# facebookresearch/mbrl-lib

Hardware: AMD Instinct MI355X
Metric: candidate-steps/sec (pop×particles×horizon / plan) per CEM iter; plans/sec (higher is better)
Workload: dtype f32

## Files before the change

### __graft_entry__.py

```python
import os
import subprocess
import sys

ROOT = os.path.dirname(os.path.abspath(__file__))
PKG = os.path.join(ROOT, "mbrl-lib_amd")
CSRC = os.path.join(PKG, "csrc")
LIB = os.path.join(PKG, "hipets", "libhipets.so")
BUILDINFO = os.path.join(PKG, "hipets", "libhipets.buildinfo.json")
OBJDIR = os.path.join(PKG, "build")
HIPCC = os.environ.get("HIPCC", "/opt/rocm/bin/hipcc")
HOST_UNITS = ["train.hip", "plan.hip", "rollout.hip", "model.hip", "policy.hip", "sac.hip", "value.hip", "ensemble.hip", "policy_rollout.hip", "replay.hip", "comm.hip", "engine.hip"]
UNITS = ["rollout_r3.hip", "rollout_r4_gen.hip", "rollout_r4_gens.hip", "rollout_r3_gen.hip", "rollout_r3_gens.hip", "rollout_r2.hip", "rollout_r2_gen.hip",
         "rollout_r2_gens.hip", "rollout_r1_gen.hip", "rollout_r1_gens.hip", "rollout_r1.hip", "rollout_r4.hip", "rollout_r2_fast.hip", "rollout_r3_fast.hip",
         "rollout_r1_fast.hip", "planet.hip"] + HOST_UNITS + ["rollout_r4_fast.hip"]
FLAGS = ["--offload-arch=gfx950", "-O3", "-std=c++17", "-ffp-contract=off", "-fPIC", "-Wno-pass-failed"]


def _sources():
    return sorted(os.path.join(CSRC, f) for f in os.listdir(CSRC)) + [os.path.join(ROOT, "include", "hipets.h")]


def source_digest(extra_flags=()):
    import hashlib

# ... 108 lines not shown
            if asm and op.split("_")[0] in ("global", "buffer", "flat", "scratch") and re.search(r"_store_dwordx[34]", op):
                store_data = regs(ops[1]) if op.startswith(("global", "flat", "scratch")) else regs(ops[0])
            recent.append((nop, regs(ops[0]) if (op.startswith("v_") and ops) else set(), line, store_data))
        if len(recent) > 8:
            del recent[0]
        return inflight

    def undrained(inflight, recent):
        ws = 0
        for nop, written, _, store in reversed(recent[-3:]):
            if ws >= 2:
                break
            if nop is not None:
                ws += nop
                continue
            if written or store:
                return True
            ws += 1
        return bool(inflight)

    edges = []
    kernel, inflight, recent = "?", [], []
    for kind, text, asm in prog:
        if kind == "kernel":
            kernel, inflight, recent = text, [], []
        elif kind == "ins":
            inflight = step(kernel, text, asm, inflight, recent, True, "")
            op = text.split()[0]
            if op.startswith("s_cbranch") or op == "s_branch":
                target = text.split()[-1]
                if target in labels and undrained(inflight, recent):
                    edges.append((kernel, target, list(inflight), list(recent)))
            if op in ("s_branch", "s_endpgm", "s_setpc_b64"):
                inflight, recent = [], []
    done = set()
    for kernel, target, inflight, recent in edges:
        key = (target, tuple(sorted((tuple(sorted(r)), c) for r, c in inflight)), tuple(t[2] for t in recent[-3:]))
        if key in done:
            continue
        done.add(key)
        walked = 0
        for kind, text, asm in prog[labels[target]:]:
            if kind == "kernel" or walked >= 16:
                break
            if kind != "ins":
                continue
            inflight = step(kernel, text, asm, inflight, recent, False, f" (reached by a branch to {target})")
            walked += 1
            if text.split()[0] in ("s_branch", "s_endpgm", "s_setpc_b64"):
                break
    unique, base_seen = [], set()
    for f in findings:
        base = f.split(" (reached by a branch")[0]
        if base not in base_seen:
            base_seen.add(base)
            unique.append(f)
    return seen, unique


def parse_kernel_resources(asm_path):
    import re

    out, cur, meta = {}, None, None
    keys = {"NumVgprs": "VGPRs", "NumAgprs": "AGPRs", "ScratchSize": "ScratchSize [bytes/lane]", "Occupancy": "Occupancy [waves/SIMD]"}
    for line in open(asm_path, errors="replace"):
        m = re.match(r"^(\S+):\s+; @", line)
        if m:
            cur = m.group(1)
            continue
        m = re.match(r"^; (NumVgprs|NumAgprs|ScratchSize|Occupancy): (\d+)", line)
        if m and cur:
            out.setdefault(cur, {})[keys[m.group(1)]] = int(m.group(2))
            continue
        m = re.match(r"^\s+\.name:\s+(\S+)", line)
        if m:
            meta = m.group(1)
            continue
        m = re.match(r"^\s+\.(sgpr|vgpr)_spill_count:\s+(\d+)", line)
        if m and meta:
            out.setdefault(meta, {})["SGPRs Spill" if m.group(1) == "sgpr" else "VGPRs Spill"] = int(m.group(2))
    return {k: v for k, v in out.items() if "VGPRs" in v and "SGPRs Spill" in v}


def build_library(out=LIB, extra_flags=(), objdir=OBJDIR, force=False):
    import json
    from concurrent.futures import ThreadPoolExecutor

    digest = source_digest(extra_flags)
    if not force and built_digest(out) == digest:
        return digest
    os.makedirs(objdir, exist_ok=True)
    objs = [os.path.join(objdir, u.replace(".hip", ".o")) for u in UNITS]

    resources = {}
    isa = {"asm_mfmas": 0, "hazards": [], "units_scanned": []}

    def compile_unit(u, o):
        cmd = [HIPCC] + FLAGS + list(extra_flags) + ["-save-temps=obj", "-c", os.path.join(CSRC, u), "-o", o]
        print("[build]", " ".join(cmd), flush=True)
        proc = subprocess.run(cmd, stderr=subprocess.PIPE, text=True)
        for line in proc.stderr.splitlines():
            if "argument unused during compilation" not in line:
                print(line, file=sys.stderr)
        if proc.returncode != 0:
            raise subprocess.CalledProcessError(proc.returncode, cmd)
        stem = os.path.basename(o)[:-2]
        for f in os.listdir(objdir):
            if (f.startswith(stem + "-") or f.startswith(stem + ".")) and f != stem + ".o":
                path = os.path.join(objdir, f)
                if f.endswith("gfx950.s"):
                    resources.update(parse_kernel_resources(path))
                    n, found = scan_isa_hazards(path)
                    isa["asm_mfmas"] += n
                    isa["hazards"] += found
                    isa["units_scanned"].append(u)
                os.remove(path)

    with ThreadPoolExecutor(max_workers=min(len(UNITS), os.cpu_count() or 1)) as ex:
        list(ex.map(lambda uo: compile_unit(*uo), zip(UNITS, objs)))
    link_extra = [f for f in extra_flags if f.startswith("-fsanitize") or f in ("-fno-gpu-sanitize", "-shared-libsan")]
    cmd = [HIPCC, "--offload-arch=gfx950", "-shared", "-fPIC"] + link_extra + objs + ["-o", out]
    print("[build]", " ".join(cmd), flush=True)
    subprocess.run(cmd, check=True)
    with open(os.path.splitext(out)[0] + ".buildinfo.json", "w") as f:
        json.dump({"source_digest": digest, "flags": FLAGS + list(extra_flags), "units": UNITS, "kernels": resources, "isa": isa}, f)
    for h in isa["hazards"][:20]:
        print("[build] ISA HAZARD:", h, file=sys.stderr)
    if isa["hazards"] and not os.environ.get("HIPETS_ALLOW_ISA_HAZARDS") and "-O1" not in extra_flags:
        raise RuntimeError(f"{len(isa['hazards'])} ISA hazard finding(s) in {out}: see {os.path.splitext(out)[0]}.buildinfo.json")
    return digest


DEBUG_LIB = os.path.join(PKG, "hipets", "libhipets_debug.so")
ASAN_LIB = os.path.join(PKG, "hipets", "libhipets_asan.so")
DEBUG_OBJDIR = os.path.join(PKG, "build_debug")
DEBUG_FLAGS = ["-O1", "-gline-tables-only", "-DHIPETS_DEBUG_BOUNDS=1"]
ASAN_FLAGS = ["-fsanitize=address", "-fno-gpu-sanitize", "-shared-libsan", "-Wno-option-ignored"]


def asan_runtime() -> str:
    out = subprocess.run([HIPCC, "--print-file-name=libclang_rt.asan-x86_64.so"], capture_output=True, text=True).stdout.strip()
    if not os.path.isabs(out) or not os.path.exists(out):
        import glob

        found = sorted(glob.glob("/opt/rocm/lib/llvm/lib/clang/*/lib/linux/libclang_rt.asan-x86_64.so"))
        out = found[-1] if found else out
    return out


def build_debug(force: bool = False) -> str:
    import json

    digest = source_digest(DEBUG_FLAGS)
    rebuilt = built_digest(DEBUG_LIB) != digest or force
    build_library(out=DEBUG_LIB, extra_flags=DEBUG_FLAGS, objdir=DEBUG_OBJDIR, force=force)
    asan_digest = source_digest(DEBUG_FLAGS + ASAN_FLAGS)
    if rebuilt or built_digest(ASAN_LIB) != asan_digest:
        from concurrent.futures import ThreadPoolExecutor

        def compile_asan(u):
            obj = os.path.join(DEBUG_OBJDIR, u.replace(".hip", "_asan.o"))
            cmd = [HIPCC] + FLAGS + DEBUG_FLAGS + ASAN_FLAGS + ["-c", os.path.join(CSRC, u), "-o", obj]
            print("[build]", " ".join(cmd), flush=True)
            subprocess.run(cmd, check=True)
            return obj

        with ThreadPoolExecutor(max_workers=min(len(HOST_UNITS), os.cpu_count() or 1)) as ex:
            objs = list(ex.map(compile_asan, HOST_UNITS))
        others = [os.path.join(DEBUG_OBJDIR, u.replace(".hip", ".o")) for u in UNITS if u not in HOST_UNITS]
        cmd = [HIPCC, "--offload-arch=gfx950", "-shared", "-fPIC", "-fsanitize=address", "-fno-gpu-sanitize", "-shared-libsan"] + objs + others + ["-o", ASAN_LIB]
        print("[build]", " ".join(cmd), flush=True)
        subprocess.run(cmd, check=True)
        with open(os.path.splitext(ASAN_LIB)[0] + ".buildinfo.json", "w") as f:
            json.dump({"source_digest": asan_digest, "flags": FLAGS + DEBUG_FLAGS + ASAN_FLAGS, "units": UNITS}, f)
    return DEBUG_LIB


def build(force: bool = False, debug: bool = True) -> None:
    build_library(force=force)
    if debug and os.environ.get("HIPETS_BUILD_DEBUG", "1") != "0":
        build_debug(force)
    build_c_client(force)
    build_fake_rccl(force)
    build_residency_harness(force)
    build_resident_heads_harness(force)
    for p in (PKG, ROOT):
        if p not in sys.path:
            sys.path.insert(0, p)
    import hipets
    from hipets import _lib

    _lib.load()
    from oracle import pets_oracle

# ... 103 lines not shown
```

### mbrl-lib_amd/csrc/gemm_f32.hpp

```cpp
#pragma once
#include <type_traits>

#include "common.hpp"
#include "rollout_types.hpp"

namespace hipets {

__device__ __forceinline__ void mfma16x16x4(const float a, const float b, f32x4& c) {
    asm volatile("v_mfma_f32_16x16x4_f32 %0, %1, %2, %0" : "+v"(c) : "v"(a), "v"(b));
}
__device__ __forceinline__ void mfma16x16x4_ra(const float a, const float b, f32x4& c) {
    asm volatile("v_mfma_f32_16x16x4_f32 %0, %1, %2, %0" : "+v"(c) : "a"(a), "v"(b));
}
__device__ __forceinline__ void mfma_drain() { asm volatile("s_nop 15" ::: "memory"); }

__device__ __forceinline__ int lds_col(int c) { return (c & ~15) | ((c & 3) << 2) | ((c >> 2) & 3); }

constexpr int kProfCountShift = 44;
struct Prof {
    long long* slot;
    long long t;
    bool on;
    __device__ __forceinline__ void mark(int phase) {
        if (on) {
            const long long now = clock64();
            slot[phase] += (now - t) + (1ll << kProfCountShift);
            t = now;
        }
    }
};

#ifndef HIPETS_LEAN_PROF
#define HIPETS_LEAN_PROF 0
#endif

template <int R, int CT, int EX>
struct GemmFrags {
    f32x4 b[CT > 0 ? CT : 1];
    f32x4 bx[EX > 0 ? EX : 1];
    f32x4 a[R];
    f32x4 ax[EX > 0 ? EX : 1];
};

using u32x4g = __attribute__((ext_vector_type(4))) unsigned;

template <int R> struct MinWavesOf { static constexpr int value = R <= 2 ? 2 : 1; };

#ifndef HIPETS_DEBUG_BOUNDS
#define HIPETS_DEBUG_BOUNDS 0
#endif
#if HIPETS_DEBUG_BOUNDS
__host__ __device__ inline void hipets_bound_fail(const int line) {
#if defined(__HIP_DEVICE_COMPILE__)
    printf("hipets: bound violated at gemm_f32.hpp / rollout.hpp line %d (workgroup %d, thread %d)\n", line, (int)blockIdx.x, (int)threadIdx.x);
    __builtin_trap();
#else
    (void)line;
#endif
}
#define HIPETS_BOUND(cond) do { if (!(cond)) hipets_bound_fail(__LINE__); } while (0)
#else
#define HIPETS_BOUND(cond) ((void)0)
#endif

struct ResHead {
    f32x4 b[3], bx[3], bv[3], bvx[3];
};
__device__ __forceinline__ void res_load(f32x4& dst, const float* const p) { asm volatile("global_load_dwordx4 %0, %1, off" : "=a"(dst) : "v"(p) : "memory"); }
__device__ __forceinline__ void res_pin(f32x4& v) { asm volatile("" : "+a"(v)); }

struct NoTail {};
struct FusedSlot {
    float mxA, mxB, mnA, mnB, pA, pB;
    double nmA, nmB, nsA, nsB;
    int rid, ndA, ndB;
    float n0, n1;
};
template <class P, class D, class F, class G>
struct TailStages {
    P prep;
    D draw;
    F unit;
    G finish;
};
template <class P, class D, class F, class G>
__device__ __forceinline__ TailStages<P, D, F, G> make_tail(P p, D d, F f, G g) { return TailStages<P, D, F, G>{p, d, f, g}; }

__device__ __forceinline__ f32x4 silu4(const f32x4 a) {
    using f32x2 = __attribute__((ext_vector_type(2))) float;
    const f32x2 k = {-1.44269504088896340736f, -1.44269504088896340736f}, one = {1.0f, 1.0f};
    const f32x2 lo = {a[0], a[1]}, hi = {a[2], a[3]};
    f32x2 tl = lo * k, th = hi * k;
    tl[0] = __builtin_amdgcn_exp2f(tl[0]); tl[1] = __builtin_amdgcn_exp2f(tl[1]);
    th[0] = __builtin_amdgcn_exp2f(th[0]); th[1] = __builtin_amdgcn_exp2f(th[1]);
    tl = tl + one; th = th + one;
    tl[0] = __builtin_amdgcn_rcpf(tl[0]); tl[1] = __builtin_amdgcn_rcpf(tl[1]);
    th[0] = __builtin_amdgcn_rcpf(th[0]); th[1] = __builtin_amdgcn_rcpf(th[1]);
    const f32x2 yl = lo * tl, yh = hi * th;
    return f32x4{yl[0], yl[1], yh[0], yh[1]};
}

constexpr int kKsSlots = 4;
struct KsArgs {
    const float* part_in;
    float* part_out;
    int tile;
    int k0, n;
    int wave;
};

template <int R, int CT, int EX, int ACT, class TL = NoTail, int LD = -1, bool SPL = false, int KCS = -1, int KS = 0, int RES = 0>
__device__ __forceinline__ void wave_gemm(const float* __restrict__ in, float* __restrict__ out, const int ld_rt,
                                          const float* __restrict__ W, const float* __restrict__ bias, const int KC_rt,
                                          const int tail_steps, const int c_first, const Extras ex,
                                          const bool apply_act, const int act, const float slope, const int lane,
                                          Prof& prof, const TL* tl = nullptr, const int ldi_rt = 0, const KsArgs* ks = nullptr,
                                          const ResHead* rh = nullptr, const int rsel = 0) {
    static_assert(!RES || (LD > 0 && KS == 0 && R >= 3 && CT <= 3 && EX <= 3), "resident heads: shape-specialised one-wave-per-SIMD instances");
    constexpr int CTn = CT > 0 ? CT : 1;
    constexpr int EXn = EX > 0 ? EX : 1;
    constexpr bool KSI = (KS & 1) != 0, KSO = (KS & 2) != 0;
    static_assert(!KS || (R == 1 && LD > 0), "k-split: one-tile shape-specialised instances, rolled k loop");
    static_assert(!KSO || (std::is_same<TL, NoTail>::value && EX == 0 && !SPL), "k-split producer: a hidden op");
    f32x4 acc[CTn][R];
    f32x4 accx[EXn];
    const int ld = LD > 0 ? LD : ld_rt;
    const int ldi = ldi_rt > 0 ? ldi_rt : ld;
    const int KC = KCS > 0 ? KCS : KC_rt;

    const int exc[kMaxExtras] = {ex.c0, ex.c1, ex.c2, ex.c3};
    const int exr[kMaxExtras] = {ex.r0, ex.r1, ex.r2, ex.r3};
    unsigned woff[CTn], wxoff[EXn];
    int axoff[EXn];
#pragma unroll
    for (int ct = 0; ct < CT; ++ct) woff[ct] = (unsigned)(((c_first + kWaves * ct) * KC * 64 + lane) * 16);
#pragma unroll
    for (int e = 0; e < EX; ++e) {
        wxoff[e] = (unsigned)((exc[e] * KC * 64 + lane) * 16);
        axoff[e] = exr[e] * 16 * ldi;
    }
    const float* ap = in + (lane & 15) * ldi + 4 * (lane >> 4);
    f32x4 bv[CTn], bvx[EXn];
    if constexpr (!RES) {
#pragma unroll
    for (int ct = 0; ct < CT; ++ct) bv[ct] = *reinterpret_cast<const f32x4*>(bias + (c_first + kWaves * ct) * 16 + 4 * (lane >> 4));
#pragma unroll
    for (int e = 0; e < EX; ++e) bvx[e] = *reinterpret_cast<const f32x4*>(bias + exc[e] * 16 + 4 * (lane >> 4));
    }
    const unsigned long long wbits = reinterpret_cast<unsigned long long>(W);
    const unsigned long long wuni = ((unsigned long long)(unsigned)__builtin_amdgcn_readfirstlane((int)(wbits >> 32)) << 32) |
                                    (unsigned long long)(unsigned)__builtin_amdgcn_readfirstlane((int)(unsigned)wbits);
    const __amdgpu_buffer_rsrc_t wrsrc = __builtin_amdgcn_make_buffer_rsrc(reinterpret_cast<float*>(wuni), 0, 0x7FFFFFFF, 0x00020000);
    auto wload = [&](const unsigned voff, const int kk) __attribute__((always_inline)) {
        const u32x4g v = __builtin_amdgcn_raw_buffer_load_b128(wrsrc, (int)voff, kk * 1024, 0);
        f32x4 r;
        __builtin_memcpy(&r, &v, 16);
        return r;
    };
    auto load = [&](GemmFrags<R, CT, EX>& f, const int kk) __attribute__((always_inline)) {
#pragma unroll
        for (int ct = 0; ct < CT; ++ct) f.b[ct] = wload(woff[ct], kk);
#pragma unroll
        for (int e = 0; e < EX; ++e) f.bx[e] = wload(wxoff[e], kk);
#pragma unroll
        for (int r = 0; r < R; ++r) f.a[r] = *reinterpret_cast<const f32x4*>(ap + r * 16 * ldi + kk * 16);
#pragma unroll
        for (int e = 0; e < EX; ++e) f.ax[e] = *reinterpret_cast<const f32x4*>(ap + axoff[e] + kk * 16);
    };
    constexpr bool kSplit = (CT * R + EX) == 1;
    constexpr bool kSplitAll = SPL && !kSplit;
    f32x4 acc_odd = f32x4{0.f, 0.f, 0.f, 0.f};
    f32x4 acco[CTn][R], accxo[EXn];
#pragma unroll
    for (int ct = 0; ct < CTn; ++ct)
#pragma unroll
        for (int r = 0; r < R; ++r) acco[ct][r] = f32x4{0.f, 0.f, 0.f, 0.f};
#pragma unroll
    for (int e = 0; e < EXn; ++e) accxo[e] = f32x4{0.f, 0.f, 0.f, 0.f};
    auto kstep = [&](const GemmFrags<R, CT, EX>& f, const int s) __attribute__((always_inline)) {
        asm volatile("s_nop 1");
        if constexpr (kSplit) {
            f32x4& dst = (s & 1) ? acc_odd : (CT ? acc[0][0] : accx[0]);
            if constexpr (CT) mfma16x16x4(f.b[0][s], f.a[0][s], dst);
            else mfma16x16x4(f.bx[0][s], f.ax[0][s], dst);
        } else if constexpr (kSplitAll) {
#pragma unroll
            for (int ct = 0; ct < CT; ++ct)
#pragma unroll
                for (int r = 0; r < R; ++r) mfma16x16x4(f.b[ct][s], f.a[r][s], (s & 1) ? acco[ct][r] : acc[ct][r]);
#pragma unroll
            for (int e = 0; e < EX; ++e) mfma16x16x4(f.bx[e][s], f.ax[e][s], (s & 1) ? accxo[e] : accx[e]);
        } else {
#pragma unroll
            for (int ct = 0; ct < CT; ++ct)
#pragma unroll
                for (int r = 0; r < R; ++r) mfma16x16x4(f.b[ct][s], f.a[r][s], acc[ct][r]);
#pragma unroll
            for (int e = 0; e < EX; ++e) mfma16x16x4(f.bx[e][s], f.ax[e][s], accx[e]);
        }
    };
    auto compute = [&](const GemmFrags<R, CT, EX>& f) __attribute__((always_inline)) {
#pragma unroll
        for (int s = 0; s < 4; ++s) kstep(f, s);
    };
    constexpr bool kIL = LD > 0;
    constexpr int kNU = CT * R + EX;
    constexpr int kNL = CT + EX + (CT > 0 ? R : 0) + EX;
    static_assert(4 * kNU >= kNL + 1, "every load needs its own slot behind an MFMA");
    auto load_one = [&](GemmFrags<R, CT, EX>& g, const int kk, const int i) __attribute__((always_inline)) {
        __builtin_amdgcn_sched_barrier(0);
        if (i < CT) g.b[i < CT ? i : 0] = wload(woff[i < CT ? i : 0], kk);
        else if (i < CT + EX) g.bx[i - CT] = wload(wxoff[i - CT], kk);
        else if (CT > 0 && i < CT + EX + R) g.a[i - CT - EX] = *reinterpret_cast<const f32x4*>(ap + (i - CT - EX) * 16 * ldi + kk * 16);
        else {
            const int e = i - CT - EX - (CT > 0 ? R : 0);
            g.ax[e] = *reinterpret_cast<const f32x4*>(ap + axoff[e] + kk * 16);
        }
        __builtin_amdgcn_sched_barrier(0);
    };
    auto mfma_unit = [&](const GemmFrags<R, CT, EX>& f, const int s, const int u) __attribute__((always_inline)) {
        if constexpr (kSplit) {
            f32x4& dst = (s & 1) ? acc_odd : (CT ? acc[0][0] : accx[0]);
            if constexpr (CT) mfma16x16x4(f.b[0][s], f.a[0][s], dst);
            else mfma16x16x4(f.bx[0][s], f.ax[0][s], dst);
        } else if (u < CT * R) {
            const int ct = u / R, r = u - ct * R;
            if constexpr (kSplitAll) mfma16x16x4(f.b[ct][s], f.a[r][s], (s & 1) ? acco[ct][r] : acc[ct][r]);
            else mfma16x16x4(f.b[ct][s], f.a[r][s], acc[ct][r]);
        } else {
            const int e = u - CT * R;
            if constexpr (kSplitAll) mfma16x16x4(f.bx[e][s], f.ax[e][s], (s & 1) ? accxo[e] : accx[e]);
            else mfma16x16x4(f.bx[e][s], f.ax[e][s], accx[e]);
        }
    };
    auto loads_behind = [&](GemmFrags<R, CT, EX>& g, const int kk_next, const int m1) __attribute__((always_inline)) {
#pragma unroll
        for (int j = 0; j < kNL; ++j)
            if (((j + 1) * 4 * kNU) / (kNL + 1) == m1) load_one(g, kk_next, j);
    };
    auto compute_il = [&](const GemmFrags<R, CT, EX>& f, GemmFrags<R, CT, EX>& g, const int kk_next) __attribute__((always_inline)) {
#pragma unroll
        for (int ks = 0; ks < 4; ++ks) {
            asm volatile("s_nop 1");
#pragma unroll
            for (int ct = 0; ct < CT; ++ct)
#pragma unroll
                for (int r = 0; r < R; ++r) {
                    mfma_unit(f, ks, ct * R + r);
                    loads_behind(g, kk_next, ks * kNU + ct * R + r + 1);
                }
#pragma unroll
            for (int e = 0; e < EX; ++e) {
                mfma_unit(f, ks, CT * R + e);
                loads_behind(g, kk_next, ks * kNU + CT * R + e + 1);
            }
        }
    };
    auto drain_all = [&]() __attribute__((always_inline)) {
        mfma_drain();
#pragma unroll
        for (int ct = 0; ct < CT; ++ct)
#pragma unroll
            for (int r = 0; r < R; ++r) asm volatile("" : "+v"(acc[ct][r]));
#pragma unroll
        for (int e = 0; e < EX; ++e) asm volatile("" : "+v"(accx[e]));
        asm volatile("" : "+v"(acc_odd));
        if constexpr (kSplitAll) {
#pragma unroll
            for (int ct = 0; ct < CT; ++ct)
#pragma unroll
                for (int r = 0; r < R; ++r) asm volatile("" : "+v"(acco[ct][r]));
#pragma unroll
            for (int e = 0; e < EX; ++e) asm volatile("" : "+v"(accxo[e]));
        }
    };
    auto compute_tail = [&](const GemmFrags<R, CT, EX>& f) __attribute__((always_inline)) {
        switch (tail_steps) {
            case 1: kstep(f, 0); drain_all(); break;
            case 2: kstep(f, 0); kstep(f, 1); drain_all(); break;
            case 3: kstep(f, 0); kstep(f, 1); kstep(f, 2); drain_all(); break;
            default: kstep(f, 0); kstep(f, 1); kstep(f, 2); kstep(f, 3); drain_all(); break;
        }
    };

    f32x4 ks_p[kWaves], ks_b[kKsSlots], ks_a[kKsSlots], ks_bias = f32x4{0.f, 0.f, 0.f, 0.f};
    if constexpr (KSI) {
#pragma unroll
        for (int w = 0; w < kWaves; ++w) ks_p[w] = *reinterpret_cast<const f32x4*>(ks->part_in + (w * 64 + lane) * 4);
    }
    if constexpr (KSO) {
        const unsigned xoff = (unsigned)((ks->tile * KC * 64 + lane) * 16);
        ks_bias = *reinterpret_cast<const f32x4*>(bias + ks->tile * 16 + 4 * (lane >> 4));
#pragma unroll
        for (int j = 0; j < kKsSlots; ++j) {
            const int c = j < ks->n ? ks->k0 + j : 0;
            ks_b[j] = wload(xoff, c);
            ks_a[j] = *reinterpret_cast<const f32x4*>(ap + c * 16);
        }
    }
    GemmFrags<R, CT, EX> f0, f1;
    if constexpr (RES) {
#pragma unroll
        for (int r = 0; r < (CT > 0 ? R : 0); ++r) f0.a[r] = *reinterpret_cast<const f32x4*>(ap + r * 16 * ldi);
#pragma unroll
        for (int e = 0; e < EX; ++e) f0.ax[e] = *reinterpret_cast<const f32x4*>(ap + axoff[e]);
    } else {
        load(f0, 0);
    }
    constexpr bool kTriple = KS != 0 && KCS > 0 && LD > 0;
    static_assert(!KS || KCS <= 0 || kTriple, "k-split ops with a static chunk count run the three-set loop");
    if constexpr (kTriple) load(f1, KCS > 1 ? 1 : 0);
    if constexpr (!RES) {
#pragma unroll
    for (int ct = 0; ct < CTn; ++ct)
#pragma unroll
        for (int r = 0; r < R; ++r) acc[ct][r] = CT > 0 ? bv[ct] : f32x4{0.f, 0.f, 0.f, 0.f};
#pragma unroll
    for (int e = 0; e < EXn; ++e) accx[e] = EX > 0 ? bvx[e] : f32x4{0.f, 0.f, 0.f, 0.f};
    }
    auto pin = [](f32x4& v) __attribute__((always_inline)) { asm volatile("" : "+v"(v)); };
    if constexpr (!RES) {
#pragma unroll
    for (int ct = 0; ct < CTn; ++ct)
#pragma unroll
        for (int r = 0; r < R; ++r) {
            if constexpr (CT > 0) pin(acc[ct][r]);
            if constexpr (CT > 0 && kSplitAll) pin(acco[ct][r]);
        }
#pragma unroll
    for (int e = 0; e < EXn; ++e) {
        if constexpr (EX > 0) pin(accx[e]);
        if constexpr (EX > 0 && kSplitAll) pin(accxo[e]);
    }
    if constexpr (kSplit) pin(acc_odd);
    prof.mark(14);
    }
    f32x4 a_last = f32x4{0.f, 0.f, 0.f, 0.f};
    if constexpr (KSI) {
        static_assert(ACT == HIPETS_ACT_SILU, "k-split instances are SiLU instances");
        a_last = silu4((ks_p[0] + ks_p[1]) + (ks_p[2] + ks_p[3]));
    }
    f32x4 ks_e = f32x4{0.f, 0.f, 0.f, 0.f}, ks_o = f32x4{0.f, 0.f, 0.f, 0.f};
    if constexpr (KSO) {
        ks_e = ks_bias * (ks->wave == 0 ? 1.0f : 0.0f);
#pragma unroll
        for (int j = 0; j < kKsSlots; ++j) ks_b[j] = ks_b[j] * (j < ks->n ? 1.0f : 0.0f);
        if constexpr (KSI) {
            HIPETS_BOUND(KC >= 13 && KC <= 16);
            ks_a[kKsSlots - 1] = a_last;
        }
        pin(ks_e);
        pin(ks_o);
#pragma unroll
        for (int j = 0; j < kKsSlots; ++j) {
            pin(ks_b[j]);
            pin(ks_a[j]);
        }
#pragma unroll
        for (int j = 0; j < kKsSlots; ++j)
#pragma unroll
            for (int s_ = 0; s_ < 4; ++s_) {
                asm volatile("s_nop 1");
                mfma16x16x4(ks_b[j][s_], ks_a[j][s_], (s_ & 1) ? ks_o : ks_e);
            }
        prof.mark(7);
    }
    if constexpr (RES != 0) {
        auto acc_init = [&](const f32x4* const b, const f32x4* const bx) __attribute__((always_inline)) {
#pragma unroll
            for (int ct = 0; ct < CTn; ++ct)
#pragma unroll
                for (int r = 0; r < R; ++r) acc[ct][r] = CT > 0 ? b[ct] : f32x4{0.f, 0.f, 0.f, 0.f};
#pragma unroll
            for (int e = 0; e < EXn; ++e) accx[e] = EX > 0 ? bx[e] : f32x4{0.f, 0.f, 0.f, 0.f};
        };
        auto pin_acc = [&]() __attribute__((always_inline)) {
#pragma unroll
            for (int ct = 0; ct < CTn; ++ct)
#pragma unroll
                for (int r = 0; r < R; ++r) {
                    if constexpr (CT > 0) pin(acc[ct][r]);
                    if constexpr (CT > 0 && kSplitAll) pin(acco[ct][r]);
                }
#pragma unroll
            for (int e = 0; e < EXn; ++e) {
                if constexpr (EX > 0) pin(accx[e]);
                if constexpr (EX > 0 && kSplitAll) pin(accxo[e]);
            }
            if constexpr (kSplit) pin(acc_odd);
        };
        auto mfma_unit_h = [&](const ResHead& h, const GemmFrags<R, CT, EX>& f, const int s, const int u) __attribute__((always_inline)) {
            if constexpr (kSplit) {
                f32x4& dst = (s & 1) ? acc_odd : (CT ? acc[0][0] : accx[0]);
                if constexpr (CT) mfma16x16x4_ra(h.b[0][s], f.a[0][s], dst);
                else mfma16x16x4_ra(h.bx[0][s], f.ax[0][s], dst);
            } else if (u < CT * R) {
                const int ct = u / R, r = u - ct * R;
                if constexpr (kSplitAll) mfma16x16x4_ra(h.b[ct][s], f.a[r][s], (s & 1) ? acco[ct][r] : acc[ct][r]);
                else mfma16x16x4_ra(h.b[ct][s], f.a[r][s], acc[ct][r]);
            } else {
                const int e = u - CT * R;
                if constexpr (kSplitAll) mfma16x16x4_ra(h.bx[e][s], f.ax[e][s], (s & 1) ? accxo[e] : accx[e]);
                else mfma16x16x4_ra(h.bx[e][s], f.ax[e][s], accx[e]);
            }
        };
        auto head = [&](const ResHead& h) __attribute__((always_inline)) {
            acc_init(h.bv, h.bvx);
            pin_acc();
            prof.mark(14);
            auto kstep_h = [&](const int s) __attribute__((always_inline)) {
                asm volatile("s_nop 1");
#pragma unroll
                for (int u = 0; u < kNU; ++u) mfma_unit_h(h, f0, s, u);
            };
            if (KC >= 2) {
#pragma unroll
                for (int ks_ = 0; ks_ < 4; ++ks_) {
                    asm volatile("s_nop 1");
#pragma unroll
                    for (int u = 0; u < kNU; ++u) {
                        mfma_unit_h(h, f0, ks_, u);
                        loads_behind(f1, 1, ks_ * kNU + u + 1);
                    }
                }
                if constexpr (RES == 3 || KCS <= 0) drain_all();
            } else {
                switch (tail_steps) {
                    case 1: kstep_h(0); drain_all(); break;
                    case 2: kstep_h(0); kstep_h(1); drain_all(); break;
                    case 3: kstep_h(0); kstep_h(1); kstep_h(2); drain_all(); break;
                    default: kstep_h(0); kstep_h(1); kstep_h(2); kstep_h(3); drain_all(); break;
                }
            }
        };
        auto rest = [&]() __attribute__((always_inline)) {
            if (KC < 2) return;
            int kk = 1;
            if constexpr (KCS > 0) {
#pragma unroll
                for (int k2 = 1; k2 + 2 < KCS; k2 += 2) {
                    compute_il(f1, f0, k2 + 1);
                    compute_il(f0, f1, k2 + 2);
                }
                constexpr int kEndR = KCS >= 3 ? 1 + ((KCS - 2) / 2) * 2 : 1;
                if constexpr (kEndR + 1 < KCS) {
                    compute_il(f1, f0, kEndR + 1);
                    compute_tail(f0);
                } else {
                    compute_tail(f1);
                }
            } else {
                for (; kk + 2 < KC; kk += 2) {
                    compute_il(f1, f0, kk + 1);
                    compute_il(f0, f1, kk + 2);
                }
                if (kk > 1) drain_all();
                if (kk + 1 < KC) {
                    compute_il(f1, f0, kk + 1);
                    compute_tail(f0);
                } else {
                    compute_tail(f1);
                }
            }
        };
        if constexpr (RES == 1) {
            head(rh[0]);
        } else {
            switch (rsel) {
                case 0: head(rh[0]); break;
                case 1: head(rh[1]); break;
                default: head(rh[2]); break;
            }
        }
        rest();
    } else if constexpr (KCS > 0 && !kTriple) {
        constexpr int kEnd = KCS >= 2 ? ((KCS - 1) / 2) * 2 : 0;
#pragma unroll
        for (int kk = 0; kk + 2 < KCS; kk += 2) {
            if constexpr (kIL) {
                compute_il(f0, f1, kk + 1);
                compute_il(f1, f0, kk + 2);
            } else {
                load(f1, kk + 1);
                __builtin_amdgcn_sched_barrier(0);
                compute(f0);
                __builtin_amdgcn_sched_barrier(0);
                load(f0, kk + 2);
                __builtin_amdgcn_sched_barrier(0);
                compute(f1);
                __builtin_amdgcn_sched_barrier(0);
            }
        }
        if constexpr (kEnd + 1 < KCS) {
            if constexpr (kIL) {
                compute_il(f0, f1, kEnd + 1);
            } else {
                load(f1, kEnd + 1);
                __builtin_amdgcn_sched_barrier(0);
                compute(f0);
                __builtin_amdgcn_sched_barrier(0);
            }
            compute_tail(f1);
        } else {
            compute_tail(f0);
        }
    } else if constexpr (kTriple) {
        GemmFrags<R, CT, EX> f2;
        auto last_frag = [&](GemmFrags<R, CT, EX>& f) __attribute__((always_inline)) {
            if constexpr (KSI) {
                if constexpr (CT > 0) f.a[0] = a_last;
#pragma unroll
                for (int e = 0; e < EX; ++e) f.ax[e] = a_last;
                if constexpr (CT > 0) pin(f.a[0]);
#pragma unroll
                for (int e = 0; e < EX; ++e) pin(f.ax[e]);
            }
        };
        constexpr int kEnd3 = KCS >= 3 ? ((KCS - 1) / 3) * 3 : 0;
        constexpr int kRem = KCS - kEnd3;
#pragma nounroll
        for (int kk = 0; kk + 3 < KCS; kk += 3) {
            compute_il(f0, f2, kk + 2);
            compute_il(f1, f0, kk + 3);
            compute_il(f2, f1, min(kk + 4, KCS - 1));
        }
        drain_all();
        if constexpr (kRem == 1) {
            last_frag(f0);
            compute_tail(f0);
        } else if constexpr (kRem == 2) {
            compute(f0);
            drain_all();
            last_frag(f1);
            compute_tail(f1);
        } else {
            compute_il(f0, f2, kEnd3 + 2);
            compute(f1);
            drain_all();
            last_frag(f2);
            compute_tail(f2);
        }
    } else {
        int kk = 0;
        for (; kk + 2 < KC; kk += 2) {
            if constexpr (kIL) {
                compute_il(f0, f1, kk + 1);
                compute_il(f1, f0, kk + 2);
            } else {
                load(f1, kk + 1);
                __builtin_amdgcn_sched_barrier(0);
                compute(f0);
                __builtin_amdgcn_sched_barrier(0);
                load(f0, kk + 2);
                __builtin_amdgcn_sched_barrier(0);
                compute(f1);
                __builtin_amdgcn_sched_barrier(0);
            }
        }
        if (KS != 0 || kk > 0) drain_all();
        auto last_frag = [&](GemmFrags<R, CT, EX>& f) __attribute__((always_inline)) {
            if constexpr (KSI) {
                if constexpr (CT > 0) f.a[0] = a_last;
#pragma unroll
                for (int e = 0; e < EX; ++e) f.ax[e] = a_last;
                if constexpr (CT > 0) pin(f.a[0]);
#pragma unroll
                for (int e = 0; e < EX; ++e) pin(f.ax[e]);
            }
        };
        if (kk + 1 < KC) {
            if constexpr (kIL) {
                compute_il(f0, f1, kk + 1);
            } else {
                load(f1, kk + 1);
                __builtin_amdgcn_sched_barrier(0);
                compute(f0);
                __builtin_amdgcn_sched_barrier(0);
            }
            if constexpr (KS != 0) drain_all();
            last_frag(f1);
            compute_tail(f1);
        } else {
            last_frag(f0);
            compute_tail(f0);
        }
    }
    constexpr int kNUt = CT * R + EX;
    constexpr int kTailGroup = 4;
    FusedSlot slots[kTailGroup];
    auto unit_c = [&](const int u) __attribute__((always_inline)) { return u < CT * R ? c_first + kWaves * (u / R) : exc[(u >= CT * R && u < kNUt) ? u - CT * R : 0]; };
    auto unit_r = [&](const int u) __attribute__((always_inline)) { return u < CT * R ? u % R : exr[(u >= CT * R && u < kNUt) ? u - CT * R : 0]; };
    if constexpr (!std::is_same<TL, NoTail>::value) {
#pragma unroll
        for (int k = 0; k < kTailGroup; ++k)
            if (k < kNUt) tl->prep(slots[k < kNUt ? k : 0], unit_c(k), unit_r(k));
    }
    if constexpr (kSplit) {
        mfma_drain();
        if constexpr (CT) acc[0][0] += acc_odd;
        else accx[0] += acc_odd;
    }
    if constexpr (kSplitAll) {
        drain_all();
#pragma unroll
        for (int ct = 0; ct < CT; ++ct)
#pragma unroll
            for (int r = 0; r < R; ++r) acc[ct][r] += acco[ct][r];
#pragma unroll
        for (int e = 0; e < EX; ++e) accx[e] += accxo[e];
    }
    mfma_drain();
    __builtin_amdgcn_sched_barrier(0);
    prof.mark(11);
    if constexpr (!std::is_same<TL, NoTail>::value) {
#pragma unroll
        for (int g = 0; g < (kNUt + kTailGroup - 1) / kTailGroup; ++g) {
            if (g > 0) {
#pragma unroll
                for (int k = 0; k < kTailGroup; ++k) {
                    const int u = g * kTailGroup + k;
                    if (u < kNUt) tl->prep(slots[k], unit_c(u), unit_r(u));
                }
            }
            static_assert(kTailGroup % 2 == 0, "the draw stage pairs the units of a group");
#pragma unroll
            for (int k = 0; k < kTailGroup; k += 2) {
                const int u = g * kTailGroup + k;
                if (u + 1 < kNUt) tl->draw(slots[k], slots[k + 1], unit_c(u), unit_c(u + 1), true);
                else if (u < kNUt) tl->draw(slots[k], slots[k], unit_c(u), unit_c(u), false);
#pragma unroll
                for (int kk = k; kk < k + 2; ++kk) {
                    const int uu = g * kTailGroup + kk;
                    if (uu < CT * R) tl->unit(slots[kk], acc[(uu < CT * R ? uu : 0) / R][(uu < CT * R ? uu : 0) % R], unit_c(uu), unit_r(uu));
                    else if (uu < kNUt) tl->unit(slots[kk], accx[(uu >= CT * R && uu < kNUt) ? uu - CT * R : 0], unit_c(uu), unit_r(uu));
                }
            }
        }
        tl->finish();
        prof.mark(9);
        return;
    }

    if constexpr (KSO) {
        asm volatile("" : "+v"(ks_e));
        asm volatile("" : "+v"(ks_o));
        *reinterpret_cast<f32x4*>(ks->part_out + (ks->wave * 64 + lane) * 4) = ks_e + ks_o;
    }
    auto store = [&](auto actfn) __attribute__((always_inline)) {
        const int j = lane & 15, g4 = 4 * (lane >> 4);
        HIPETS_BOUND(c_first >= 0 && (CT == 0 || (c_first + kWaves * (CT - 1)) * 16 + g4 + 3 < ld) && KC >= 1 && KC * 16 <= ldi);
#pragma unroll
        for (int ct = 0; ct < CT; ++ct) {
            const int col = (c_first + kWaves * ct) * 16 + g4;
#pragma unroll
            for (int r = 0; r < R; ++r) *reinterpret_cast<f32x4*>(out + (r * 16 + j) * ld + col) = actfn(acc[ct][r]);
        }
#pragma unroll
        for (int e = 0; e < EX; ++e) *reinterpret_cast<f32x4*>(out + (exr[e] * 16 + j) * ld + exc[e] * 16 + g4) = actfn(accx[e]);
    };
    auto each = [](auto f) {
        return [f](const f32x4 a) {
            f32x4 v;
#pragma unroll
            for (int i = 0; i < 4; ++i) v[i] = f(a[i]);
            return v;
        };
    };
    if (!apply_act) {
        store([](const f32x4 a) { return a; });
    } else {
        switch (ACT >= 0 ? ACT : act) {
            case HIPETS_ACT_SILU: store([](const f32x4 a) { return silu4(a); }); break;
            case HIPETS_ACT_RELU: store(each([](float x) { return x < 0.0f ? 0.0f : x; })); break;
            case HIPETS_ACT_LEAKY_RELU: store(each([slope](float x) { return x > 0.0f ? x : slope * x; })); break;
            case HIPETS_ACT_TANH: store(each([](float x) { return tanhf(x); })); break;
            default: store(each([](float x) { return __builtin_amdgcn_rcpf(1.0f + __builtin_amdgcn_exp2f(x * -1.44269504088896340736f)); })); break;
        }
    }
    prof.mark(13);
}

template <int R, int CT, int ACT, bool SPL = false>
__device__ __forceinline__ void wave_gemm_ex(int nex, const float* in, float* out, int ld, const float* W,
                                             const float* bias, int KC, int tail_steps, int c_first, const Extras ex,
                                             bool apply_act, int act, float slope, int lane, Prof& prof) {
    constexpr int kMaxEx = (3 * R + kWaves - 1) / kWaves;
    switch (nex) {
        case 0:
            if constexpr (CT > 0) wave_gemm<R, CT, 0, ACT, NoTail, -1, SPL>(in, out, ld, W, bias, KC, tail_steps, c_first, ex, apply_act, act, slope, lane, prof);
            break;
        case 1: wave_gemm<R, CT, 1, ACT, NoTail, -1, SPL>(in, out, ld, W, bias, KC, tail_steps, c_first, ex, apply_act, act, slope, lane, prof); break;
        case 2:
            if constexpr (kMaxEx >= 2) wave_gemm<R, CT, 2, ACT, NoTail, -1, SPL>(in, out, ld, W, bias, KC, tail_steps, c_first, ex, apply_act, act, slope, lane, prof);
            break;
// ... 119 lines not shown
```

Measured before the change: 294.1 million.

## Replace tail-step switch with scalar-predicated inline-asm MFMA k-steps and fork loop by parity

For straight (static LD, single-wave, no k-split) GEMMs, the runtime switch over tail_steps is replaced by inline-asm blocks that skip each k-step with a scalar compare-and-branch on a uniform SGPR. The runtime-KC loop is forked into odd and even paths with separately pinned accumulator initialisations. The intent is to stop the compiler from duplicating code per branch and emitting long v_mov runs that shuffle accumulators between MFMAs. The build script also gains an assembly scan that counts v_mov_b64 and mov runs between MFMAs per rollout kernel. The hand-written asm adds hazard and correctness risk, and it only covers the shapes listed in its table.

```diff
diff --git a/__graft_entry__.py b/__graft_entry__.py
--- a/__graft_entry__.py
+++ b/__graft_entry__.py
@@ -214,6 +214,48 @@
     return {k: v for k, v in out.items() if "VGPRs" in v and "SGPRs Spill" in v}
 
 
+MOV_RUN = 8
+
+
+def count_accumulator_moves(asm_path):
+    import re
+
+    out, cur = {}, None
+    for line in open(asm_path, errors="replace"):
+        m = re.match(r"^(\S+):\s+; @", line)
+        if m:
+            cur = m.group(1) if "rollout_kernel" in m.group(1) else None
+            if cur:
+                out[cur] = {"v_mov_b64": 0, "mov_runs": 0}
+                run = pending = 0
+                seen_mfma = False
+            continue
+        if cur is None:
+            continue
+        m = re.match(r"^; codeLenInByte = (\d+)", line)
+        if m:
+            out[cur]["codeLenInByte"] = int(m.group(1))
+            cur = None
+            continue
+        text = line.split(";")[0].strip()
+        if not text or text.startswith(".") or text.endswith(":"):
+            continue
+        op = text.split()[0]
+        if op.startswith("v_mov_b64"):
+            out[cur]["v_mov_b64"] += 1
+        if op.startswith(("v_mov_b64", "v_mov_b32")):
+            run += 1
+            continue
+        if run >= MOV_RUN:
+            pending += 1
+        run = 0
+        if op.startswith("v_mfma"):
+            if seen_mfma:
+                out[cur]["mov_runs"] += pending
+            pending, seen_mfma = 0, True
+    return out
+
+
 def build_library(out=LIB, extra_flags=(), objdir=OBJDIR, force=False):
     import json
     from concurrent.futures import ThreadPoolExecutor
@@ -242,6 +284,9 @@
                 path = os.path.join(objdir, f)
                 if f.endswith("gfx950.s"):
                     resources.update(parse_kernel_resources(path))
+                    for kernel, moves in count_accumulator_moves(path).items():
+                        if kernel in resources:
+                            resources[kernel].update(moves)
                     n, found = scan_isa_hazards(path)
                     isa["asm_mfmas"] += n
                     isa["hazards"] += found
diff --git a/mbrl-lib_amd/csrc/gemm_f32.hpp b/mbrl-lib_amd/csrc/gemm_f32.hpp
--- a/mbrl-lib_amd/csrc/gemm_f32.hpp
+++ b/mbrl-lib_amd/csrc/gemm_f32.hpp
@@ -68,6 +68,69 @@
 };
 __device__ __forceinline__ void res_load(f32x4& dst, const float* const p) { asm volatile("global_load_dwordx4 %0, %1, off" : "=a"(dst) : "v"(p) : "memory"); }
 __device__ __forceinline__ void res_pin(f32x4& v) { asm volatile("" : "+a"(v)); }
+
+#define HIPETS_KT_MF(C, B, A) "v_mfma_f32_16x16x4_f32 %[" #C "], %[" #B "], %[" #A "], %[" #C "]\n\t"
+#define HIPETS_KT_COL3(ct) HIPETS_KT_MF(c##ct##0, b##ct, a0) HIPETS_KT_MF(c##ct##1, b##ct, a1) HIPETS_KT_MF(c##ct##2, b##ct, a2)
+#define HIPETS_KT_COL4(ct) HIPETS_KT_COL3(ct) HIPETS_KT_MF(c##ct##3, b##ct, a3)
+#define HIPETS_KT_EX(e) HIPETS_KT_MF(x##e, bx##e, ax##e)
+#define HIPETS_KT_ACC3(ct) [c##ct##0] "+v"(*c[ct][0]), [c##ct##1] "+v"(*c[ct][1]), [c##ct##2] "+v"(*c[ct][2])
+#define HIPETS_KT_ACC4(ct) HIPETS_KT_ACC3(ct), [c##ct##3] "+v"(*c[ct][3])
+#define HIPETS_KT_XACC(e) [x##e] "+v"(*x[e])
+#define HIPETS_KT_A3 [a0] "v"(a[0]), [a1] "v"(a[1]), [a2] "v"(a[2])
+#define HIPETS_KT_A4 HIPETS_KT_A3, [a3] "v"(a[3])
+#define HIPETS_KT_B(WC, ct) [b##ct] WC(b[ct])
+#define HIPETS_KT_XIN(WC, e) [bx##e] WC(bx[e]), [ax##e] "v"(ax[e])
+#define HIPETS_KT_ASM(BODY, OUTS, INS)                                                                                        \
+    asm volatile("s_cmp_le_i32 %[n], %[s]\n\ts_cbranch_scc1 .Lhipets_kt%=\n\ts_nop 1\n\t" BODY ".Lhipets_kt%=:" \
+                 : OUTS : INS, [n] "s"(n), [s] "n"(S) : "scc")
+#define HIPETS_KT_COMMA ,
+#define HIPETS_KT_SHAPES(WC)                                                                                                                        \
+    if constexpr (R == 3 && NC == 3 && NE == 1)                                                                                                     \
+        HIPETS_KT_ASM(HIPETS_KT_COL3(0) HIPETS_KT_COL3(1) HIPETS_KT_COL3(2) HIPETS_KT_EX(0),                                                        \
+                      HIPETS_KT_ACC3(0) HIPETS_KT_COMMA HIPETS_KT_ACC3(1) HIPETS_KT_COMMA HIPETS_KT_ACC3(2) HIPETS_KT_COMMA HIPETS_KT_XACC(0),      \
+                      HIPETS_KT_B(WC, 0) HIPETS_KT_COMMA HIPETS_KT_B(WC, 1) HIPETS_KT_COMMA HIPETS_KT_B(WC, 2) HIPETS_KT_COMMA HIPETS_KT_A3         \
+                          HIPETS_KT_COMMA HIPETS_KT_XIN(WC, 0));                                                                                    \
+    else if constexpr (R == 3 && NC == 3 && NE == 0)                                                                                                \
+        HIPETS_KT_ASM(HIPETS_KT_COL3(0) HIPETS_KT_COL3(1) HIPETS_KT_COL3(2),                                                                        \
+                      HIPETS_KT_ACC3(0) HIPETS_KT_COMMA HIPETS_KT_ACC3(1) HIPETS_KT_COMMA HIPETS_KT_ACC3(2),                                        \
+                      HIPETS_KT_B(WC, 0) HIPETS_KT_COMMA HIPETS_KT_B(WC, 1) HIPETS_KT_COMMA HIPETS_KT_B(WC, 2) HIPETS_KT_COMMA HIPETS_KT_A3);       \
+    else if constexpr (R == 3 && NC == 1 && NE == 1)                                                                                                \
+        HIPETS_KT_ASM(HIPETS_KT_COL3(0) HIPETS_KT_EX(0), HIPETS_KT_ACC3(0) HIPETS_KT_COMMA HIPETS_KT_XACC(0),                                       \
+                      HIPETS_KT_B(WC, 0) HIPETS_KT_COMMA HIPETS_KT_A3 HIPETS_KT_COMMA HIPETS_KT_XIN(WC, 0));                                        \
+    else if constexpr (R == 3 && NC == 1 && NE == 2)                                                                                                \
+        HIPETS_KT_ASM(HIPETS_KT_COL3(0) HIPETS_KT_EX(0) HIPETS_KT_EX(1), HIPETS_KT_ACC3(0) HIPETS_KT_COMMA HIPETS_KT_XACC(0) HIPETS_KT_COMMA HIPETS_KT_XACC(1), \
+                      HIPETS_KT_B(WC, 0) HIPETS_KT_COMMA HIPETS_KT_A3 HIPETS_KT_COMMA HIPETS_KT_XIN(WC, 0) HIPETS_KT_COMMA HIPETS_KT_XIN(WC, 1));   \
+    else if constexpr (R == 4 && NC == 2 && NE == 0)                                                                                                \
+        HIPETS_KT_ASM(HIPETS_KT_COL4(0) HIPETS_KT_COL4(1), HIPETS_KT_ACC4(0) HIPETS_KT_COMMA HIPETS_KT_ACC4(1),                                     \
+                      HIPETS_KT_B(WC, 0) HIPETS_KT_COMMA HIPETS_KT_B(WC, 1) HIPETS_KT_COMMA HIPETS_KT_A4);                                          \
+    else if constexpr (R == 4 && NC == 1 && NE == 0)                                                                                                \
+        HIPETS_KT_ASM(HIPETS_KT_COL4(0), HIPETS_KT_ACC4(0), HIPETS_KT_B(WC, 0) HIPETS_KT_COMMA HIPETS_KT_A4);                                       \
+    else if constexpr (R == 4 && NC == 1 && NE == 1)                                                                                                \
+        HIPETS_KT_ASM(HIPETS_KT_COL4(0) HIPETS_KT_EX(0), HIPETS_KT_ACC4(0) HIPETS_KT_COMMA HIPETS_KT_XACC(0),                                       \
+                      HIPETS_KT_B(WC, 0) HIPETS_KT_COMMA HIPETS_KT_A4 HIPETS_KT_COMMA HIPETS_KT_XIN(WC, 0));                                        \
+    else if constexpr (R == 4 && NC == 1 && NE == 2)                                                                                                \
+        HIPETS_KT_ASM(HIPETS_KT_COL4(0) HIPETS_KT_EX(0) HIPETS_KT_EX(1), HIPETS_KT_ACC4(0) HIPETS_KT_COMMA HIPETS_KT_XACC(0) HIPETS_KT_COMMA HIPETS_KT_XACC(1), \
+                      HIPETS_KT_B(WC, 0) HIPETS_KT_COMMA HIPETS_KT_A4 HIPETS_KT_COMMA HIPETS_KT_XIN(WC, 0) HIPETS_KT_COMMA HIPETS_KT_XIN(WC, 1));   \
+    else if constexpr (NC == 0 && NE == 1)                                                                                                          \
+        HIPETS_KT_ASM(HIPETS_KT_EX(0), HIPETS_KT_XACC(0), HIPETS_KT_XIN(WC, 0));                                                                    \
+    else if constexpr (NC == 0 && NE == 2)                                                                                                          \
+        HIPETS_KT_ASM(HIPETS_KT_EX(0) HIPETS_KT_EX(1), HIPETS_KT_XACC(0) HIPETS_KT_COMMA HIPETS_KT_XACC(1),                                         \
+                      HIPETS_KT_XIN(WC, 0) HIPETS_KT_COMMA HIPETS_KT_XIN(WC, 1));                                                                   \
+    else if constexpr (NC == 0 && NE == 3)                                                                                                          \
+        HIPETS_KT_ASM(HIPETS_KT_EX(0) HIPETS_KT_EX(1) HIPETS_KT_EX(2), HIPETS_KT_XACC(0) HIPETS_KT_COMMA HIPETS_KT_XACC(1) HIPETS_KT_COMMA HIPETS_KT_XACC(2), \
+                      HIPETS_KT_XIN(WC, 0) HIPETS_KT_COMMA HIPETS_KT_XIN(WC, 1) HIPETS_KT_COMMA HIPETS_KT_XIN(WC, 2));                              \
+    else                                                                                                                                            \
+        static_assert(R < 0, "conditional k-step: a (row tiles, column tiles, extras) share the shape tables do not produce")
+template <int R, int NC, int NE, int S, bool WA>
+__device__ __forceinline__ void mfma_kstep_if(const int n, f32x4* const (&c)[NC > 0 ? NC : 1][R], f32x4* const (&x)[NE > 0 ? NE : 1],
+                                              const float (&b)[NC > 0 ? NC : 1], const float (&a)[R], const float (&bx)[NE > 0 ? NE : 1],
+                                              const float (&ax)[NE > 0 ? NE : 1]) {
+    if constexpr (WA) {
+        HIPETS_KT_SHAPES("a");
+    } else {
+        HIPETS_KT_SHAPES("v");
+    }
+}
 
 struct NoTail {};
 struct FusedSlot {
@@ -127,6 +190,8 @@
     const int ld = LD > 0 ? LD : ld_rt;
     const int ldi = ldi_rt > 0 ? ldi_rt : ld;
     const int KC = KCS > 0 ? KCS : KC_rt;
+    constexpr bool kStraight = LD > 0 && MinWavesOf<R>::value == 1 && KS == 0;
+    const int tail_sgpr = kStraight ? __builtin_amdgcn_readfirstlane(tail_steps) : tail_steps;
 
     const int exc[kMaxExtras] = {ex.c0, ex.c1, ex.c2, ex.c3};
     const int exr[kMaxExtras] = {ex.r0, ex.r1, ex.r2, ex.r3};
@@ -274,7 +339,60 @@
             for (int e = 0; e < EX; ++e) asm volatile("" : "+v"(accxo[e]));
         }
     };
+    auto kstep_if = [&](const auto& wb, const auto& wbx, const GemmFrags<R, CT, EX>& f, auto sc, auto wa, const int n) __attribute__((always_inline)) {
+        constexpr int S = decltype(sc)::value;
+        constexpr bool WA = decltype(wa)::value;
+        constexpr bool odd = (S & 1) != 0;
+        float ea[R] = {}, eax[EXn] = {}, ebx[EXn] = {};
+        f32x4* px[EXn] = {};
+#pragma unroll
+        for (int r = 0; r < (CT > 0 ? R : 0); ++r) ea[r] = f.a[r][S];
+#pragma unroll
+        for (int e = 0; e < EX; ++e) {
+            eax[e] = f.ax[e][S];
+            ebx[e] = wbx[e][S];
+            px[e] = (kSplitAll && odd) ? &accxo[e] : ((kSplit && odd) ? &acc_odd : &accx[e]);
+        }
+        if constexpr (kSplit && CT > 0) {
+            static_assert(R < 0, "conditional k-step: one strided unit");
+        } else if constexpr (2 * (CT * R + EX) + CT + (CT > 0 ? R : 0) + 2 * EX + 1 <= 30) {
+            f32x4* pc[CTn][R] = {};
+            float eb[CTn] = {};
+#pragma unroll
+            for (int ct = 0; ct < CT; ++ct) {
+                eb[ct] = wb[ct][S];
+#pragma unroll
+                for (int r = 0; r < R; ++r) pc[ct][r] = (kSplitAll && odd) ? &acco[ct][r] : &acc[ct][r];
+            }
+            mfma_kstep_if<R, CT, EX, S, WA>(n, pc, px, eb, ea, ebx, eax);
+        } else {
+            static_assert(CT == 3, "two statements: the widest share is three column tiles and the extra units");
+            f32x4* p01[2][R];
+            f32x4* p2[1][R];
+            float e01[2], e2[1];
+#pragma unroll
+            for (int ct = 0; ct < 2; ++ct) {
+                e01[ct] = wb[ct][S];
+#pragma unroll
+                for (int r = 0; r < R; ++r) p01[ct][r] = (kSplitAll && odd) ? &acco[ct][r] : &acc[ct][r];
+            }
+            e2[0] = wb[2][S];
+#pragma unroll
+            for (int r = 0; r < R; ++r) p2[0][r] = (kSplitAll && odd) ? &acco[2][r] : &acc[2][r];
+            f32x4* pnone[1] = {nullptr};
+            const float enone[1] = {0.f};
+            mfma_kstep_if<R, 2, 0, S, WA>(n, p01, pnone, e01, ea, enone, enone);
+            mfma_kstep_if<R, 1, EX, S, WA>(n, p2, px, e2, ea, ebx, eax);
+        }
+    };
     auto compute_tail = [&](const GemmFrags<R, CT, EX>& f) __attribute__((always_inline)) {
+        if constexpr (kStraight) {
+            kstep(f, 0);
+            kstep_if(f.b, f.bx, f, std::integral_constant<int, 1>{}, std::false_type{}, tail_sgpr);
+            kstep_if(f.b, f.bx, f, std::integral_constant<int, 2>{}, std::false_type{}, tail_sgpr);
+            kstep_if(f.b, f.bx, f, std::integral_constant<int, 3>{}, std::false_type{}, tail_sgpr);
+            return;
+        }
         switch (tail_steps) {
             case 1: kstep(f, 0); drain_all(); break;
             case 2: kstep(f, 0); kstep(f, 1); drain_all(); break;
@@ -310,31 +428,35 @@
     constexpr bool kTriple = KS != 0 && KCS > 0 && LD > 0;
     static_assert(!KS || KCS <= 0 || kTriple, "k-split ops with a static chunk count run the three-set loop");
     if constexpr (kTriple) load(f1, KCS > 1 ? 1 : 0);
-    if constexpr (!RES) {
-#pragma unroll
-    for (int ct = 0; ct < CTn; ++ct)
-#pragma unroll
-        for (int r = 0; r < R; ++r) acc[ct][r] = CT > 0 ? bv[ct] : f32x4{0.f, 0.f, 0.f, 0.f};
-#pragma unroll
-    for (int e = 0; e < EXn; ++e) accx[e] = EX > 0 ? bvx[e] : f32x4{0.f, 0.f, 0.f, 0.f};
-    }
     auto pin = [](f32x4& v) __attribute__((always_inline)) { asm volatile("" : "+v"(v)); };
-    if constexpr (!RES) {
-#pragma unroll
-    for (int ct = 0; ct < CTn; ++ct)
-#pragma unroll
-        for (int r = 0; r < R; ++r) {
-            if constexpr (CT > 0) pin(acc[ct][r]);
-            if constexpr (CT > 0 && kSplitAll) pin(acco[ct][r]);
-        }
-#pragma unroll
-    for (int e = 0; e < EXn; ++e) {
-        if constexpr (EX > 0) pin(accx[e]);
-        if constexpr (EX > 0 && kSplitAll) pin(accxo[e]);
-    }
-    if constexpr (kSplit) pin(acc_odd);
-    prof.mark(14);
-    }
+    auto pin_in = [](f32x4& v, auto body) __attribute__((always_inline)) {
+        if constexpr (decltype(body)::value == 0) asm volatile("" : "+v"(v));
+        else asm volatile("; body %1" : "+v"(v) : "n"(decltype(body)::value));
+    };
+    auto acc_from_bias = [&](auto body) __attribute__((always_inline)) {
+#pragma unroll
+        for (int ct = 0; ct < CTn; ++ct)
+#pragma unroll
+            for (int r = 0; r < R; ++r) acc[ct][r] = CT > 0 ? bv[ct] : f32x4{0.f, 0.f, 0.f, 0.f};
+#pragma unroll
+        for (int e = 0; e < EXn; ++e) accx[e] = EX > 0 ? bvx[e] : f32x4{0.f, 0.f, 0.f, 0.f};
+#pragma unroll
+        for (int ct = 0; ct < CTn; ++ct)
+#pragma unroll
+            for (int r = 0; r < R; ++r) {
+                if constexpr (CT > 0) pin_in(acc[ct][r], body);
+                if constexpr (CT > 0 && kSplitAll) pin_in(acco[ct][r], body);
+            }
+#pragma unroll
+        for (int e = 0; e < EXn; ++e) {
+            if constexpr (EX > 0) pin_in(accx[e], body);
+            if constexpr (EX > 0 && kSplitAll) pin_in(accxo[e], body);
+        }
+        if constexpr (kSplit) pin_in(acc_odd, body);
+        prof.mark(14);
+    };
+    constexpr bool kForked = kStraight && KCS <= 0;
+    if constexpr (!RES && !kForked) acc_from_bias(std::integral_constant<int, 0>{});
     f32x4 a_last = f32x4{0.f, 0.f, 0.f, 0.f};
     if constexpr (KSI) {
         static_assert(ACT == HIPETS_ACT_SILU, "k-split instances are SiLU instances");
@@ -374,20 +496,20 @@
 #pragma unroll
             for (int e = 0; e < EXn; ++e) accx[e] = EX > 0 ? bx[e] : f32x4{0.f, 0.f, 0.f, 0.f};
         };
-        auto pin_acc = [&]() __attribute__((always_inline)) {
+        auto pin_acc = [&](auto body) __attribute__((always_inline)) {
 #pragma unroll
             for (int ct = 0; ct < CTn; ++ct)
 #pragma unroll
                 for (int r = 0; r < R; ++r) {
-                    if constexpr (CT > 0) pin(acc[ct][r]);
-                    if constexpr (CT > 0 && kSplitAll) pin(acco[ct][r]);
+                    if constexpr (CT > 0) pin_in(acc[ct][r], body);
+                    if constexpr (CT > 0 && kSplitAll) pin_in(acco[ct][r], body);
                 }
 #pragma unroll
             for (int e = 0; e < EXn; ++e) {
-                if constexpr (EX > 0) pin(accx[e]);
-                if constexpr (EX > 0 && kSplitAll) pin(accxo[e]);
-            }
-            if constexpr (kSplit) pin(acc_odd);
+                if constexpr (EX > 0) pin_in(accx[e], body);
+                if constexpr (EX > 0 && kSplitAll) pin_in(accxo[e], body);
+            }
+            if constexpr (kSplit) pin_in(acc_odd, body);
         };
         auto mfma_unit_h = [&](const ResHead& h, const GemmFrags<R, CT, EX>& f, const int s, const int u) __attribute__((always_inline)) {
             if constexpr (kSplit) {
@@ -404,75 +526,84 @@
                 else mfma16x16x4_ra(h.bx[e][s], f.ax[e][s], accx[e]);
             }
         };
-        auto head = [&](const ResHead& h) __attribute__((always_inline)) {
+        auto head_init = [&](const ResHead& h, auto body) __attribute__((always_inline)) {
             acc_init(h.bv, h.bvx);
-            pin_acc();
+            pin_acc(body);
             prof.mark(14);
-            auto kstep_h = [&](const int s) __attribute__((always_inline)) {
+        };
+        auto head_full = [&](const ResHead& h) __attribute__((always_inline)) {
+#pragma unroll
+            for (int ks_ = 0; ks_ < 4; ++ks_) {
                 asm volatile("s_nop 1");
 #pragma unroll
-                for (int u = 0; u < kNU; ++u) mfma_unit_h(h, f0, s, u);
+                for (int u = 0; u < kNU; ++u) {
+                    mfma_unit_h(h, f0, ks_, u);
+                    loads_behind(f1, 1, ks_ * kNU + u + 1);
+                }
+            }
+        };
+        if constexpr (KCS > 0) {
+            static_assert(KCS >= 2, "a hidden width of more than one chunk");
+            auto head = [&](const ResHead& h) __attribute__((always_inline)) {
+                head_init(h, std::integral_constant<int, 0>{});
+                head_full(h);
+                if constexpr (RES == 3) drain_all();
             };
-            if (KC >= 2) {
-#pragma unroll
-                for (int ks_ = 0; ks_ < 4; ++ks_) {
-                    asm volatile("s_nop 1");
-#pragma unroll
-                    for (int u = 0; u < kNU; ++u) {
-                        mfma_unit_h(h, f0, ks_, u);
-                        loads_behind(f1, 1, ks_ * kNU + u + 1);
-                    }
+            if constexpr (RES == 1) {
+                head(rh[0]);
+            } else {
+                switch (rsel) {
+                    case 0: head(rh[0]); break;
+                    case 1: head(rh[1]); break;
+                    default: head(rh[2]); break;
                 }
-                if constexpr (RES == 3 || KCS <= 0) drain_all();
+            }
+#pragma unroll
+            for (int k2 = 1; k2 + 2 < KCS; k2 += 2) {
+                compute_il(f1, f0, k2 + 1);
+                compute_il(f0, f1, k2 + 2);
+            }
+            constexpr int kEndR = KCS >= 3 ? 1 + ((KCS - 2) / 2) * 2 : 1;
+            if constexpr (kEndR + 1 < KCS) {
+                compute_il(f1, f0, kEndR + 1);
+                compute_tail(f0);
             } else {
-                switch (tail_steps) {
-                    case 1: kstep_h(0); drain_all(); break;
-                    case 2: kstep_h(0); kstep_h(1); drain_all(); break;
-                    case 3: kstep_h(0); kstep_h(1); kstep_h(2); drain_all(); break;
-                    default: kstep_h(0); kstep_h(1); kstep_h(2); kstep_h(3); drain_all(); break;
+                compute_tail(f1);
+            }
+        } else {
+            static_assert(RES == 1, "one head");
+            const ResHead& h = rh[0];
+            if (KC < 2) {
+                head_init(h, std::integral_constant<int, 1>{});
+                asm volatile("s_nop 1");
+#pragma unroll
+                for (int u = 0; u < kNU; ++u) mfma_unit_h(h, f0, 0, u);
+                kstep_if(h.b, h.bx, f0, std::integral_constant<int, 1>{}, std::true_type{}, tail_sgpr);
+                kstep_if(h.b, h.bx, f0, std::integral_constant<int, 2>{}, std::true_type{}, tail_sgpr);
+                kstep_if(h.b, h.bx, f0, std::integral_constant<int, 3>{}, std::true_type{}, tail_sgpr);
+                drain_all();
+            } else if ((KC & 1) == 0) {
+                head_init(h, std::integral_constant<int, 2>{});
+                head_full(h);
+                for (int kk = 1; kk + 2 < KC; kk += 2) {
+                    compute_il(f1, f0, kk + 1);
+                    compute_il(f0, f1, kk + 2);
                 }
-            }
-        };
-        auto rest = [&]() __attribute__((always_inline)) {
-            if (KC < 2) return;
-            int kk = 1;
-            if constexpr (KCS > 0) {
-#pragma unroll
-                for (int k2 = 1; k2 + 2 < KCS; k2 += 2) {
-                    compute_il(f1, f0, k2 + 1);
-                    compute_il(f0, f1, k2 + 2);
-                }
-                constexpr int kEndR = KCS >= 3 ? 1 + ((KCS - 2) / 2) * 2 : 1;
-                if constexpr (kEndR + 1 < KCS) {
-                    compute_il(f1, f0, kEndR + 1);
-                    compute_tail(f0);
-                } else {
-                    compute_tail(f1);
-                }
+                compute_tail(f1);
+                drain_all();
             } else {
+                head_init(h, std::integral_constant<int, 3>{});
+                head_full(h);
+                int kk = 1;
                 for (; kk + 2 < KC; kk += 2) {
                     compute_il(f1, f0, kk + 1);
                     compute_il(f0, f1, kk + 2);
                 }
-                if (kk > 1) drain_all();
-                if (kk + 1 < KC) {
-                    compute_il(f1, f0, kk + 1);
-                    compute_tail(f0);
-                } else {
-                    compute_tail(f1);
-                }
-            }
-        };
-        if constexpr (RES == 1) {
-            head(rh[0]);
-        } else {
-            switch (rsel) {
-                case 0: head(rh[0]); break;
-                case 1: head(rh[1]); break;
-                default: head(rh[2]); break;
-            }
-        }
-        rest();
+                compute_il(f1, f0, kk + 1);
+                compute_tail(f0);
+                drain_all();
+            }
+        }
     } else if constexpr (KCS > 0 && !kTriple) {
         constexpr int kEnd = KCS >= 2 ? ((KCS - 1) / 2) * 2 : 0;
 #pragma unroll
@@ -540,6 +671,26 @@
             last_frag(f2);
             compute_tail(f2);
         }
+    } else if constexpr (kStraight) {
+        if (KC & 1) {
+            acc_from_bias(std::integral_constant<int, 1>{});
+            int kk = 0;
+            for (; kk + 2 < KC; kk += 2) {
+                compute_il(f0, f1, kk + 1);
+                compute_il(f1, f0, kk + 2);
+            }
+            compute_tail(f0);
+            drain_all();
+        } else {
+            acc_from_bias(std::integral_constant<int, 2>{});
+            compute_il(f0, f1, 1);
+            for (int kk = 1; kk + 2 < KC; kk += 2) {
+                compute_il(f1, f0, kk + 1);
+                compute_il(f0, f1, kk + 2);
+            }
+            compute_tail(f1);
+            drain_all();
+        }
     } else {
         int kk = 0;
         for (; kk + 2 < KC; kk += 2) {
@@ -609,7 +760,7 @@
 #pragma unroll
         for (int e = 0; e < EX; ++e) accx[e] += accxo[e];
     }
-    mfma_drain();
+    if constexpr (!kForked) mfma_drain();
     __builtin_amdgcn_sched_barrier(0);
     prof.mark(11);
     if constexpr (!std::is_same<TL, NoTail>::value) {
```

Result: faster. 299.9 million (median of 6 runs) (+2.0%).
